# hasindu2008/cornetto

Measured on AMD Instinct MI355X. Metric: Gbases/s scanned (telowin+sdust+boringbits), higher is better.
Workload: dtype u8/u16 integer

## Files before the change

### cornetto_amd/csrc/common.hpp

```cpp
#pragma once
#include <hip/hip_runtime.h>

#include <cstdarg>
#include <cstdint>
#include <cstdio>
#include <cstdlib>
#include <cstring>
#include <algorithm>
#include <atomic>
#include <string>
#include <utility>
#include <vector>

#include "../../include/cornetto_accel.h"

#ifndef CN_STREAM_PRIO
#define CN_STREAM_PRIO 3
#endif

inline std::atomic<uint64_t> cn_uid_counter{1};

struct cornetto_accel {
    int device = 0;
    std::string tf_lut_key;
    const void *tf_lut_ptr = nullptr;
    uint64_t tf_bm_uid = 0;
    const void *tf_bm_ptr = nullptr;
    size_t tf_bm_words = 0;

    hipStream_t stream = nullptr;
    bool own_stream = false;
    hipStream_t stream2 = nullptr;
// ... 13 lines not shown
    Ws dev[64];
    Ws pin[32];
    int sd_slots = 0;
    int sd_cus = 0;
    int sift_per_cu = 0;
    int sift_per_cu_default = -1;
    int lazy = 0;
    hipStream_t copy_stream = nullptr;
    hipEvent_t ev_cp = nullptr;
    bool copies_pending = false;
    volatile int boost = 0;
    volatile unsigned long long launch_seq = 0;
    hipEvent_t ev3 = nullptr;
    int share = 100;
    int sd_stats = 0;
    struct SdPend {
        int state = 0;
        const void *a = nullptr;
        int32_t T = 0, W = 0;
        void *of = nullptr;
        size_t m_cap = 0, n_cap = 0, cap = 0;
        int64_t key = 0, n_done = 0;
        bool walk_pending = false;
    } sd_pend;
    unsigned long long sd_last[256] = {0};
    uint32_t scan_epoch = 0, scan_tickets = 0;
    uint32_t st_epoch = 0, st_tickets = 0;
    size_t te_cap = 0;
    int timing = 2;
};

static inline void *cn_ws(cornetto_accel_t *h, int slot, size_t bytes)
{
    cornetto_accel::Ws &w = h->dev[slot];
    if (bytes == 0) bytes = 16;
    if (w.bytes >= bytes) return w.p;
#ifdef CN_WS_ASYNC
    if (w.p) (void)hipFreeAsync(w.p, h->stream);
    w.p = nullptr;
    w.bytes = 0;
    const size_t want = bytes + bytes / 8;
    if (hipMallocAsync(&w.p, want, h->stream) == hipSuccess) w.bytes = want;
    else w.p = nullptr;
    return w.p;
#else
    if (w.p) (void)hipFree(w.p);
    w.p = nullptr;
// ... 296 lines not shown
```

### cornetto_amd/csrc/internal.hpp

```cpp
#pragma once
#include "common.hpp"

int cn_cov_prepare_impl(cornetto_accel_t *h, cornetto_cov_t *c, int32_t w, int32_t inc, uint64_t sums[3]);

struct CnCovSpec {
    bool queued = false;
    cornetto_regpk_t *o = nullptr;
    size_t n_copy = 0, cap = 0;
    unsigned long long *p_cnt = nullptr;
    uint32_t *p_cf = nullptr;
    int64_t key = 0;
};
int cn_cov_spec_queue(cornetto_accel_t *h, cornetto_cov_t *c, int32_t lo, int32_t hi, float low_mq, int32_t edge_len, int32_t min_ctg_len, int boring,
                      unsigned long long *p_cnt, CnCovSpec *S);
int cn_cov_spec_finish(cornetto_accel_t *h, cornetto_cov_t *c, CnCovSpec *S, cornetto_regpk_t **recs, int64_t *n_recs, int64_t **ctg_first);
int cn_cov_select_packed_impl(cornetto_accel_t *h, cornetto_cov_t *c, int32_t lo, int32_t hi, float low_mq, int32_t edge_len, int32_t min_ctg_len, int boring,
                              cornetto_regpk_t **recs, int64_t *n_recs, int64_t **ctg_first);

struct CnTeloSpec {
    bool queued = false;
    cornetto_hit_t *hits = nullptr;
    size_t hit_cap = 0;
    size_t seg_cap[4] = {0, 0, 0, 0};
    int4 *p_wins = nullptr;
    size_t win_cap = 0;
    unsigned long long *p_cnt = nullptr;
};
int cn_telo_spec_queue(cornetto_accel_t *h, cornetto_asm_t *a, const char *motif, double thr_adj, unsigned long long *p_cnt, CnTeloSpec *S);
int cn_telo_spec_finish(cornetto_accel_t *h, cornetto_asm_t *a, const char *motif, double thr_adj, CnTeloSpec *S, cornetto_hit_t **hits, int64_t *n_hits,
                        cornetto_win_t **wins, int64_t *n_wins);
int cn_telo_scan_impl(cornetto_accel_t *h, const cornetto_asm_t *a, const char *motif, double thr_adj, cornetto_hit_t **hits, int64_t *n_hits, cornetto_win_t **wins,
                      int64_t *n_wins);

int cn_telo_marks_impl(cornetto_accel_t *h, const cornetto_asm_t *a, const char *motif, const unsigned long long **d_marks);
```

### cornetto_amd/csrc/runtime.hip

```cpp
#include "common.hpp"
#include <chrono>
#include <condition_variable>
#include <deque>
#include <set>
#include <thread>

#include <map>
#include <mutex>
#include <unordered_map>

namespace {
std::mutex &g_pool_mu = *new std::mutex;
std::unordered_map<void *, size_t> &g_pool_live = *new std::unordered_map<void *, size_t>;
std::multimap<size_t, void *> &g_pool_free = *new std::multimap<size_t, void *>;
std::unordered_map<void *, uint64_t> &g_pool_age = *new std::unordered_map<void *, uint64_t>;
uint64_t g_pool_clock = 0;
constexpr size_t POOL_MIN = 1u << 20;
size_t g_pool_free_bytes = 0;
constexpr size_t POOL_KEEP_BYTES = 4ull << 30;
constexpr size_t POOL_KEEP = 12;
}

namespace {
std::condition_variable &g_pre_cv = *new std::condition_variable;
// ... 114 lines not shown
        }
    }
#endif
    cornetto_accel_t *h = new (std::nothrow) cornetto_accel;
    if (!h) return CORNETTO_E_NOMEM;
    h->device = device;
    if (stream) {
        h->stream = (hipStream_t)stream;
    } else {
        if (hipStreamCreateWithFlags(&h->stream, hipStreamNonBlocking) != hipSuccess) {
            delete h;
            return CORNETTO_E_NODEVICE;
        }
        h->own_stream = true;
    }
    *out = h;
    return CORNETTO_OK;
}

void cornetto_accel_close(cornetto_accel_t *h)
{
    if (!h) return;
    (void)hipSetDevice(h->device);
    (void)hipStreamSynchronize(h->stream);
    if (h->sd_pend.state != 0 && h->sd_pend.of) cornetto_free(h->sd_pend.of);
    h->sd_pend.state = 0;
    for (auto &r : h->recs) {
        (void)hipEventDestroy(r.a);
        (void)hipEventDestroy(r.b);
    }
    for (auto e : h->pool) (void)hipEventDestroy(e);
    for (auto &w : h->dev)
        if (w.p) (void)hipFree(w.p);
    for (auto &w : h->pin)
        if (w.p) (void)hipHostFree(w.p);
    if (h->ev1) (void)hipEventDestroy(h->ev1);
    if (h->ev2) (void)hipEventDestroy(h->ev2);
    if (h->ev3) (void)hipEventDestroy(h->ev3);
    if (h->copy_stream) {
        (void)hipStreamSynchronize(h->copy_stream);
        (void)hipStreamDestroy(h->copy_stream);
    }
    if (h->ev_cp) (void)hipEventDestroy(h->ev_cp);
    if (h->stream2) {
        (void)hipStreamSynchronize(h->stream2);
        (void)hipStreamDestroy(h->stream2);
    }
    if (h->own_stream) (void)hipStreamDestroy(h->stream);
    delete h;
// ... 77 lines not shown
    if (on && !h->copy_stream) {
        CN_HIP(h, hipSetDevice(h->device));
        CN_HIP(h, hipStreamCreateWithFlags(&h->copy_stream, hipStreamNonBlocking));
        CN_HIP(h, hipEventCreateWithFlags(&h->ev_cp, hipEventDisableTiming));
    }
    return CORNETTO_OK;
}

int cornetto_accel_wait(cornetto_accel_t *h)
{
    if (!h) return CORNETTO_E_ARG;
    if (h->copies_pending) {
        CN_HIP(h, hipSetDevice(h->device));
        CN_HIP(h, hipStreamSynchronize(h->copy_stream));
        h->copies_pending = false;
    }
    return CORNETTO_OK;
}

int cornetto_accel_boost(cornetto_accel_t *h, int on)
{
    if (!h) return CORNETTO_E_ARG;
    __atomic_store_n(&h->boost, on ? 1 : 0, __ATOMIC_RELEASE);
    return CORNETTO_OK;
}

int cornetto_accel_warm(cornetto_accel_t *h, int what)
{
    if (!h) return CORNETTO_E_ARG;
    const int32_t n = 4096;
    std::vector<uint8_t> seq((size_t)n);
    std::vector<uint16_t> d((size_t)n), q((size_t)n);
    uint32_t x = 12345u;
    for (int32_t i = 0; i < n; ++i) {
        x = x * 1664525u + 1013904223u;
        seq[(size_t)i] = "ACGT"[(x >> 24) & 3];
        d[(size_t)i] = (uint16_t)(20 + ((x >> 16) & 15));
        q[(size_t)i] = (uint16_t)(d[(size_t)i] >> ((i / 700) & 1));
    }
    for (int32_t i = 100; i < 700; ++i) seq[(size_t)i] = "TTAGGG"[(i - 100) % 6];
    for (int32_t i = 1000; i < 1100; ++i) seq[(size_t)i] = 'A';
    int rc = CORNETTO_OK;
    {
        CN_HIP(h, hipSetDevice(h->device));
        const size_t nb = (size_t)1 << 20;
        void *dv = cn_ws(h, WS_FQ_CNT, nb);
// ... 72 lines not shown
static const int64_t SLACK = 256;

static int asm_finish_table(cornetto_accel_t *h, cornetto_asm_t *a)
{
    size_t n = (size_t)(a->n > 0 ? a->n : 1);
    CN_HIP(h, hipMalloc((void **)&a->d_off, n * sizeof(int64_t)));
    CN_HIP(h, hipMalloc((void **)&a->d_len, n * sizeof(int32_t)));
    if (a->n) {
        CN_HIP(h, hipMemcpyAsync(a->d_off, a->off.data(), a->n * sizeof(int64_t), hipMemcpyHostToDevice, h->stream));
        CN_HIP(h, hipMemcpyAsync(a->d_len, a->len.data(), a->n * sizeof(int32_t), hipMemcpyHostToDevice, h->stream));
    }
    CN_HIP(h, hipStreamSynchronize(h->stream));
    if (a->total >= (64ll << 20)) {
        cn_result_prewarm((size_t)(a->total / 1536 + 1) * sizeof(cornetto_hit_t));
        cn_result_prewarm((size_t)(a->total / 4096 + 1) * sizeof(cornetto_ivl_t));
    }
    return CORNETTO_OK;
}

void cornetto_asm_free(cornetto_accel_t *h, cornetto_asm_t *a)
{
    if (!a) return;
    if (h) (void)hipSetDevice(h->device);
    if (h && h->sd_pend.state != 0 && h->sd_pend.a == a) {
        if (h->sd_pend.state == 1) (void)hipStreamSynchronize(h->stream);
        if (h->sd_pend.of) cornetto_free(h->sd_pend.of);
        h->sd_pend = cornetto_accel::SdPend{};
    }
    if (a->owned) (void)hipFree(a->owned);
    if (a->d_off) (void)hipFree(a->d_off);
    if (a->d_len) (void)hipFree(a->d_len);
    if (a->d_tf_tiles) (void)hipFree(a->d_tf_tiles);
    if (a->d_tf_ct0) (void)hipFree(a->d_tf_ct0);
    if (a->d_tw_boff) (void)hipFree(a->d_tw_boff);
    if (a->d_tw_tiles) (void)hipFree(a->d_tw_tiles);
    if (a->d_sd_chunks) (void)hipFree(a->d_sd_chunks);
    a->sd_pref.release(); a->tf_pref.release(); a->tw_pref.release();
    if (a->d_sd_walk) (void)hipFree(a->d_sd_walk);
    if (a->d_sd_plan) (void)hipFree(a->d_sd_plan);
    if (a->d_wtab) (void)hipFree(a->d_wtab);
    if (a->d_wtab_base) (void)hipFree(a->d_wtab_base);
    delete a;
}

int cornetto_asm_upload(cornetto_accel_t *h, const uint8_t *const *seqs, const int64_t *lens, int32_t n,
                        cornetto_asm_t **out)
{
    if (!h || !out || n < 0 || (n > 0 && (!seqs || !lens))) return cn_fail(h, CORNETTO_E_ARG, "asm_upload: bad argument");
    *out = nullptr;
    CN_HIP(h, hipSetDevice(h->device));
// ... 275 lines not shown
```

### cornetto_amd/csrc/scan.hpp

```cpp
#pragma once
#include "common.hpp"
#include "wave.hpp"

namespace cnscan {
namespace {

constexpr int SC_THREADS = 256;
constexpr int SC_ITEMS = 16;
constexpr int SC_TILE = SC_THREADS * SC_ITEMS;

template <typename T, int THREADS>
__device__ __forceinline__ T block_excl(T s, T &total)
{
    __shared__ T wtot[THREADS / 64];
    const int lane = threadIdx.x & 63, wv = threadIdx.x >> 6;
    const T inc = cnwave::wave_incl(s, lane);
    if (lane == 63) wtot[wv] = inc;
    __syncthreads();
    T pre = inc - s;
    total = 0;
#pragma unroll
    for (int w = 0; w < THREADS / 64; ++w) {
        if (w < wv) pre += wtot[w];
        total += wtot[w];
// ... 34 lines not shown
        for (int64_t pos = tile - 1;; pos -= 64) {
            const int64_t idx = pos - lane;
            unsigned long long x;
            for (;;) {
                x = idx >= 0 ? __hip_atomic_load(&st[idx * stride], __ATOMIC_RELAXED, __HIP_MEMORY_SCOPE_AGENT) : ((2ull << 62) | tag);
                const bool ready = (x >> 62) != 0 && (x & (0x3FFFFFFFull << 32)) == tag;
                if (__builtin_amdgcn_ballot_w64(!ready) == 0) break;
                __builtin_amdgcn_s_sleep(1);
            }
            const unsigned long long incl = __builtin_amdgcn_ballot_w64((x >> 62) == 2);
            const uint32_t val = (uint32_t)x;
            if (incl) {
                const int first = __builtin_ctzll(incl);
                excl += cnwave::wave_sum(lane <= first ? val : 0u);
                break;
            }
            excl += cnwave::wave_sum(val);
        }
    }
    if (lane == 0) __hip_atomic_store(&st[tile * stride], (2ull << 62) | tag | (excl + own), __ATOMIC_RELAXED, __HIP_MEMORY_SCOPE_AGENT);
    return excl;
}

struct Outs4 {
    uint32_t *o[4];
};
struct LbArgs {
    const uint32_t *in;
    int64_t n, np;
    int stride, m;
    Outs4 outs;
    unsigned long long *state;
    uint32_t *ticket;
    uint32_t ticket_base, epoch;
    unsigned long long *total;
};

__global__ __launch_bounds__(SC_THREADS) void scan_lookback(LbArgs A)
{
    __shared__ uint32_t s_gid, s_excl;
    const int t = threadIdx.x, lane = t & 63, wv = t >> 6;
    if (t == 0) s_gid = atomicAdd(A.ticket, 1u) - A.ticket_base;
    __syncthreads();
    const int64_t gid = s_gid;
    if (gid >= (int64_t)A.m * A.np) return;
    const int q = (int)(gid / A.np);
// ... 1 lines not shown
    const int64_t base = tile * SC_TILE + (int64_t)t * SC_ITEMS;
    uint32_t v[SC_ITEMS], bt;
    uint32_t pre = tile_excl(A.in + q, base, A.n, A.stride, v, bt);
    if (wv == 0) {
        const uint32_t excl = lookback_excl(A.state + (int64_t)q * A.np, 1, tile, A.epoch, bt, lane);
        if (lane == 0) {
            s_excl = excl;
            if (A.total && tile == A.np - 1) A.total[q] = (unsigned long long)excl + bt;
        }
    }
    __syncthreads();
    pre += s_excl;
    tile_write(A.outs.o[q], base, A.n, pre, v);
}

static inline int exclusive_u32_multi(cornetto_accel_t *h, const char *name, const uint32_t *in, int64_t n, int stride, int m, uint32_t *const *outs,
                                      unsigned long long *d_total)
{
    if (n <= 0 || m <= 0) return CORNETTO_OK;
    if (m > 4) m = 4;
    Outs4 o{};
    for (int q = 0; q < m; ++q) o.o[q] = outs[q];
    const int64_t np = (n + SC_TILE - 1) / SC_TILE;
    const size_t need = 64 + (size_t)m * (size_t)np * 8;
    const bool fresh = h->dev[WS_SCAN].bytes < need || h->scan_epoch >= 0x3FFFFFFFu;
    uint8_t *ws = (uint8_t *)cn_ws(h, WS_SCAN, need);
    if (!ws) return cn_fail(h, CORNETTO_E_NOMEM, "scan: workspace allocation failed");
    const int rc = [&]() -> int {
        if (fresh) {
            CN_HIP(h, hipMemsetAsync(ws, 0, h->dev[WS_SCAN].bytes, h->stream));
            h->scan_tickets = 0;
            h->scan_epoch = 0;
        }
        const uint32_t epoch = h->scan_epoch + 1;
        LbArgs A{in, n, np, stride, m, o, reinterpret_cast<unsigned long long *>(ws + 64), reinterpret_cast<uint32_t *>(ws), h->scan_tickets, epoch, d_total};
        CN_LAUNCH(h, name, scan_lookback<<<dim3((unsigned)(m * np)), dim3(SC_THREADS), 0, h->stream>>>(A));
        h->scan_epoch = epoch;
        h->scan_tickets += (uint32_t)(m * np);
        return CORNETTO_OK;
    }();
    if (rc != CORNETTO_OK) h->dev[WS_SCAN].bytes = 0;
    return rc;
}

static inline int exclusive_u32(cornetto_accel_t *h, const char *name, const uint32_t *in, int64_t n, int stride, uint32_t *out, unsigned long long *d_total)
{
    return exclusive_u32_multi(h, name, in, n, stride, 1, &out, d_total);
}

}
}
```

### cornetto_amd/csrc/sdust.hip

```cpp
#include <algorithm>
#include <type_traits>
#include <ctime>
#include <sched.h>

#include "common.hpp"
#include "scan.hpp"
#include "tiles.hpp"
#include "ivlmerge.hpp"

namespace {

__device__ __forceinline__ int nt4_code(uint32_t c);
struct SdArgs;
struct SdChunk;
template <bool LEAN = false>
__device__ int sd_find_start(const SdArgs &A, const SdChunk ch, const uint8_t *seq);

struct SdChunk {
    int32_t ctg, start, end;
};
struct SdChunkFill {
    SdChunk *out;
    const int32_t *len;
    int32_t chunk;
    __device__ void operator()(int64_t t, int c, int64_t j) const
    {
        const int64_t s = j * chunk, e = s + chunk;
        out[t] = SdChunk{c, (int32_t)s, (int32_t)(e < len[c] ? e : len[c])};
    }
};

// ... 1290 lines not shown
    if (flag[c]) {
        pos = r * S;
    } else {
        if (S > 1u && j < H * (S - 1u)) pos = (j / (S - 1u)) * S + 1u + j % (S - 1u);
        else pos = H * S + (j - H * (S - 1u));
    }
    perm[pos] = (uint32_t)c;
}

__global__ void sdust_gather(const uint2 *in, const uint32_t *cnt, const uint32_t *dst_off, uint32_t cap, const SdChunk *chunks,
                             int32_t n_chunks, cornetto_ivl_t *dst, uint32_t dst_cap = 0xFFFFFFFFu)
{
    const int cid = blockIdx.x * blockDim.x + threadIdx.x;
    if (cid >= n_chunks) return;
    uint32_t n = cnt[cid];
    if (n == 0) return;
    if (n > cap) n = cap;
    const int32_t ctg = chunks[cid].ctg;
    const uint2 *src = in + (size_t)cid * cap;
    const uint32_t o = dst_off[cid];
    for (uint32_t i = 0; i < n && o + i < dst_cap; ++i) dst[o + i] = cornetto_ivl_t{ctg, (int32_t)src[i].x, (int32_t)src[i].y};
}

__global__ void sd_sample_count(const uint8_t *bases, const int64_t *ctg_off, const int32_t *ctg_len, unsigned long long *count)
{
    const int c = blockIdx.y;
    const int len = ctg_len[c];
    const uint8_t *seq = bases + ctg_off[c];
    unsigned n = 0;
    for (long long s = (long long)blockIdx.x * blockDim.x + threadIdx.x; s * 2048 + 64 <= len; s += (long long)gridDim.x * blockDim.x)
        n += sd_sample_heavy(SdChunk{c, (int32_t)(s * 2048), (int32_t)std::min<long long>(len, s * 2048 + 2048)}, seq);
    const unsigned long long m = sd_ballot(n != 0);
    (void)m;
    for (int d = 32; d > 0; d >>= 1) n += __shfl_down(n, d);
    if ((threadIdx.x & 63) == 0 && n) atomicAdd(count, (unsigned long long)n);
}

__global__ void sd_make_order(const uint32_t *walk, const uint32_t *iswalk, const uint32_t *rank, int32_t n_chunks, uint32_t *order)
{
    const int k = blockIdx.x * blockDim.x + threadIdx.x;
    if (k >= n_chunks) return;
    const uint32_t nw = walk[0];
    if ((uint32_t)k < nw) order[k] = walk[2 + k];
    if (!iswalk[k]) order[nw + (uint32_t)k - rank[k]] = (uint32_t)k;
}

}

extern "C" {

}

namespace {
int sd_one_go_finish(cornetto_accel_t *h, cornetto_asm_t *a, cornetto_ivl_t *of, unsigned long long *p_tot, size_t cap, size_t n_cap, size_t m_cap, int64_t key,
                     bool walk_pending, cornetto_ivl_t **ivls, int64_t *n_ivls)
{
    if (hipStreamSynchronize(h->stream) != hipSuccess) {
        cornetto_free(of);
        return cn_fail(h, CORNETTO_E_HIP, "sdust: stitch / copy back failed");
    }
    const uint32_t ovf_f = (uint32_t)(p_tot[1] & 0xFFFFFFFFull);
    const bool wtab_f = (p_tot[1] >> 32) != 0;
    const unsigned long long rows_f = p_tot[0], out_f = rows_f ? p_tot[9] : 0ull;
    if (!wtab_f && ovf_f <= cap && rows_f <= n_cap && out_f != ~0ull && out_f <= m_cap && out_f <= rows_f && (rows_f == 0 || out_f > 0)) {
        if (walk_pending) a->sd_walk_key = key;
        a->sd_est_rows = (int64_t)rows_f;
        a->sd_est_out = (int64_t)out_f;
        cn_timing_end(h);
        *ivls = of;
        *n_ivls = (int64_t)out_f;
        return 0;
    }
    cornetto_free(of);
    a->sd_est_key = -1;
    return 1;
}

int sdust_asm_impl(cornetto_accel_t *h, const cornetto_asm_t *a_in, int32_t T, int32_t W, cornetto_ivl_t **ivls, int64_t *n_ivls, const int phase)
{
    static const bool trace = CN_DEV_INT("CORNETTO_SDUST_TRACE", 0) != 0;
    struct timespec ts0;
    clock_gettime(CLOCK_MONOTONIC, &ts0);
    auto stamp = [&](const char *what) {
        if (!trace) return;
        struct timespec t;
        clock_gettime(CLOCK_MONOTONIC, &t);
        fprintf(stderr, "[sdust trace] %-22s %8.3f ms\n", what, (t.tv_sec - ts0.tv_sec) * 1e3 + (t.tv_nsec - ts0.tv_nsec) * 1e-6);
    };
    if (!h || !a_in || !ivls || !n_ivls) return cn_fail(h, CORNETTO_E_ARG, "sdust: bad argument");
    cornetto_asm_t *a = const_cast<cornetto_asm_t *>(a_in);
    *ivls = nullptr;
    *n_ivls = 0;
    if (W < 3 || W > 1026) return cn_fail(h, CORNETTO_E_UNSUPPORTED, "sdust: -w %d outside 3..1026 (the reference crashes below 3)", W);
    if (T < 0 || T > (1 << 20)) return cn_fail(h, CORNETTO_E_UNSUPPORTED, "sdust: -t %d outside 0..2^20", T);
    CN_HIP(h, hipSetDevice(h->device));
    cn_timing_begin(h);

    const int variant0 = CN_DEV_INT("CORNETTO_SDUST_VARIANT", 0);
    const bool w64_path = W - 2 <= 64 && T >= 5 && T <= 100000 && variant0 == 0;
    if (w64_path && h->sd_slots == 0) {
// ... 150 lines not shown
    const size_t nc = (size_t)a->sd_n_chunks;
    cornetto_ivl_t *o = nullptr;
    int64_t n_out = 0;
    stamp("chunk table");
    if (nc > 0) {
        const SdChunk *d_chunks = reinterpret_cast<const SdChunk *>(a->d_sd_chunks);
        uint32_t *d_cnt = (uint32_t *)cn_ws(h, WS_SD_CNT, nc * 8 + 4);
        unsigned long long *d_tot = (unsigned long long *)cn_ws(h, WS_SD_STATS, 2048 + 64 * 64);
        unsigned long long *p_tot = (unsigned long long *)cn_pin(h, PIN_SMALL, 2048);
        if (!d_cnt || !d_tot || !p_tot) return cn_fail(h, CORNETTO_E_NOMEM, "sdust: workspace allocation failed");
        uint32_t *d_off = d_cnt + nc;
        stamp("small workspaces");
        const bool env_stats = CN_DEV_INT("CORNETTO_SDUST_STATS", 0) != 0;
        const bool want_stats = env_stats || h->sd_stats != 0;
        size_t cap = (size_t)std::max<int64_t>(16, chunk / 32);
        cap = (size_t)CN_DEV_INT("CORNETTO_SDUST_CAP", (int)cap);
        if (h->dev[WS_SD_OUT].bytes / (nc * sizeof(uint2)) > cap) cap = h->dev[WS_SD_OUT].bytes / (nc * sizeof(uint2));
        unsigned long long tot = 0;
        uint2 *d_out = nullptr;
        const int64_t est_key = key * 131 + T * 1031 + W;
        const bool one_go = w64_path && sift_on && !want_stats && a->sd_est_key == est_key && a->sd_est_rows >= 0 && CN_DEV_INT("CORNETTO_SDUST_FUSED", 1);
        if (phase == 1 && !one_go)
            return CORNETTO_OK;
        for (int attempt = 0; attempt < 4; ++attempt) {
            d_out = (uint2 *)cn_ws(h, WS_SD_OUT, nc * cap * sizeof(uint2));
            if (!d_out) return cn_fail(h, CORNETTO_E_NOMEM, "sdust: workspace allocation of %zu bytes failed", nc * cap * sizeof(uint2));
            CN_HIP(h, hipMemsetAsync(d_tot, 0, 2048 + 64 * 64, h->stream));
            uint32_t *d_slots = (uint32_t *)cn_ws(h, WS_SD_OFF, (size_t)(std::max<int64_t>(sd_waves, 1) + SD_WPB) * 64 * 64 * sizeof(uint32_t));
            if (!d_slots) return cn_fail(h, CORNETTO_E_NOMEM, "sdust: workspace allocation failed");
            stamp("row + slot workspaces");
            const bool use_w64 = w64_path;
            SdArgs A{a->d_bases, a->d_off, a->d_len, d_chunks, (int32_t)nc, T, W, d_out, d_cnt, (uint32_t)cap,
                     want_stats ? d_tot + 2 : nullptr, reinterpret_cast<uint32_t *>(d_tot + 1), d_slots, nullptr,
                     reinterpret_cast<uint32_t *>(d_tot + 8), nullptr, 0, CN_DEV_INT("CORNETTO_SDUST_RUNON", 1), (int32_t)chunk, a->d_wtab, a->d_wtab_base, reinterpret_cast<uint32_t *>(d_tot + 1) + 1};
            unsigned nb = (unsigned)((nc + 63) / 64);
            bool sift_walk_pending = false;
            bool dense_pending = false;
            struct DenseJoin {
                cornetto_accel_t *h;
                bool *pending;
                ~DenseJoin() { if (*pending && h->stream2) (void)hipStreamSynchronize(h->stream2); }
            } dense_join{h, &dense_pending};
            if (use_w64 && sift_on) {
                CN_HIP(h, hipMemsetAsync(d_cnt, 0, nc * 4, h->stream));
                const uint32_t reg_cap = (uint32_t)(chunk + 128);
                const uint32_t lds_wave = sift_lds_bytes(reg_cap);
                int lmin = 1;
                while (5 * (lmin + 1) <= T && lmin < 16) ++lmin;
                const bool walk_known = a->d_sd_walk && a->sd_walk_key == key;
                const size_t walk_words = 2 + 4 * nc + 2;
                if (!walk_known) {
                    if (a->d_sd_walk) { (void)hipFree(a->d_sd_walk); a->d_sd_walk = nullptr; }
                    a->sd_walk_key = -1;
                    if (cn_obj_malloc(h, (void **)&a->d_sd_walk, walk_words * 4) != hipSuccess) return cn_fail(h, CORNETTO_E_NOMEM, "sdust: device allocation failed");
                    CN_HIP(h, hipMemsetAsync(a->d_sd_walk, 0, (2 + 2 * nc) * 4, h->stream));
                }
                uint32_t *d_wflag = a->d_sd_walk + 2 + nc, *d_wrank = d_wflag + nc, *d_worder = d_wrank + nc;
                SiftArgs S{a->d_bases, a->d_off, a->d_len, d_chunks, (int32_t)nc, T, W, lds_wave, reg_cap,
                           walk_known ? d_worder : nullptr, walk_known ? nullptr : a->d_sd_walk, walk_known ? nullptr : d_wflag,
                           reinterpret_cast<uint32_t *>(d_tot + 256), T / 10 + 1, lmin, CN_DEV_INT("CORNETTO_SIFT_ABL", 0),
                           std::min(65, std::max(1, CN_DEV_INT("CORNETTO_SIFT_DP", 24))), std::min(65, std::max(1, CN_DEV_INT("CORNETTO_SIFT_L2SKIP", 48)))};
                sift_walk_pending = !walk_known;
                SdArgs R = A;
                R.stats = want_stats ? d_tot + 200 : nullptr;
                const bool cap_default = reg_cap == SIFT_CAP_DEFAULT && !CN_DEV_INT("CORNETTO_SIFT_GENERIC", 0) && !CN_DEV_INT("CORNETTO_SIFT_ABL", 0);
                if (h->sift_per_cu == 0 || h->sift_per_cu_default != (cap_default ? 1 : 0)) {
                    int per_cu = 0;
                    const hipError_t oe = cap_default ? hipOccupancyMaxActiveBlocksPerMultiprocessor(&per_cu, sd_sift<false, SIFT_CAP_DEFAULT>, 64 * SIFT_WPB, lds_wave * SIFT_WPB)
                                                      : hipOccupancyMaxActiveBlocksPerMultiprocessor(&per_cu, sd_sift<false>, 64 * SIFT_WPB, lds_wave * SIFT_WPB);
                    if (oe != hipSuccess || per_cu < 1) per_cu = 8;
                    h->sift_per_cu = per_cu;
                    h->sift_per_cu_default = cap_default ? 1 : 0;
                }
                const int per_cu_all = std::max(1, std::min<int>(h->sift_per_cu, (int)(163840 / ((lds_wave * SIFT_WPB + 1279) / 1280 * 1280))));
                const bool free_now = __atomic_load_n(&h->boost, __ATOMIC_ACQUIRE) != 0;
                const size_t cus_n = (size_t)std::max(h->sd_cus, 1);
                const size_t slots_all = (size_t)per_cu_all * cus_n;
                const size_t slots = free_now ? slots_all : std::max<size_t>(cus_n, slots_all * (size_t)h->share / 100);
                const size_t all_blocks = (nc + SIFT_WPB - 1) / SIFT_WPB;
                const unsigned nbk = (unsigned)std::min<size_t>(all_blocks, (size_t)CN_DEV_INT("CORNETTO_SIFT_BLOCKS", (int)slots));
                const unsigned extra = (unsigned)std::min<size_t>(all_blocks > nbk ? all_blocks - nbk : 0, slots_all > slots ? slots_all - slots : 0);
                const bool may_help = phase == 0 && extra > 0 && !want_stats && h->share < CN_DEV_INT("CORNETTO_SDUST_HELP_BELOW", 70);
                if (may_help) {
                    if (!h->stream2) {
                        int pr_least = 0, pr_greatest = 0;
                        (void)hipDeviceGetStreamPriorityRange(&pr_least, &pr_greatest);
                        CN_HIP(h, hipStreamCreateWithPriority(&h->stream2, hipStreamNonBlocking, pr_greatest));
                        CN_HIP(h, hipEventCreateWithFlags(&h->ev2, hipEventDisableTiming));
                        CN_HIP(h, hipEventCreateWithFlags(&h->ev1, hipEventDisableTiming));
                    }
                    if (!h->ev3) CN_HIP(h, hipEventCreateWithFlags(&h->ev3, hipEventDisableTiming));
                    CN_HIP(h, hipEventRecord(h->ev1, h->stream));
                }
                stamp("set up");
                if (want_stats) CN_LAUNCH(h, "sdust_kernel", sd_sift<true><<<dim3(nbk), dim3(64 * SIFT_WPB), lds_wave * SIFT_WPB, h->stream>>>(S, R));
                else if (cap_default) CN_LAUNCH(h, "sdust_kernel", sd_sift<false, SIFT_CAP_DEFAULT><<<dim3(nbk), dim3(64 * SIFT_WPB), lds_wave * SIFT_WPB, h->stream>>>(S, R));
                else CN_LAUNCH(h, "sdust_kernel", sd_sift<false><<<dim3(nbk), dim3(64 * SIFT_WPB), lds_wave * SIFT_WPB, h->stream>>>(S, R));
                __atomic_fetch_add(&h->launch_seq, 1ull, __ATOMIC_RELEASE);
                if (may_help) {
                    CN_HIP(h, hipEventRecord(h->ev3, h->stream));
                    bool helped = false;
                    while (hipEventQuery(h->ev3) == hipErrorNotReady) {
                        if (!helped && __atomic_load_n(&h->boost, __ATOMIC_ACQUIRE) != 0) {
                            CN_HIP(h, hipStreamWaitEvent(h->stream2, h->ev1, 0));
                            if (cap_default) sd_sift<false, SIFT_CAP_DEFAULT><<<dim3(extra), dim3(64 * SIFT_WPB), lds_wave * SIFT_WPB, h->stream2>>>(S, R);
                            else sd_sift<false><<<dim3(extra), dim3(64 * SIFT_WPB), lds_wave * SIFT_WPB, h->stream2>>>(S, R);
                            dense_pending = true;
                            CN_HIP(h, hipGetLastError());
                            CN_HIP(h, hipEventRecord(h->ev2, h->stream2));
                            helped = true;
                        }
                        sched_yield();
                    }
                    if (helped) CN_HIP(h, hipStreamWaitEvent(h->stream, h->ev2, 0));
// ... 97 lines not shown
                if ((unsigned)sd_waves < nb) nb = (unsigned)sd_waves;
                nb = (nb + SD_WPB - 1) / SD_WPB * SD_WPB;
                if (want_stats) CN_LAUNCH(h, "sdust_kernel", sdust_w64<true><<<dim3(nb / SD_WPB), dim3(64 * SD_WPB), 0, h->stream>>>(A));
                else CN_LAUNCH(h, "sdust_kernel", sdust_w64<false><<<dim3(nb / SD_WPB), dim3(64 * SD_WPB), 0, h->stream>>>(A));
            } else if (W - 2 <= 64) {
                CN_LAUNCH(h, "sdust_kernel", sdust_kernel<64><<<dim3(nb), dim3(64), 0, h->stream>>>(A));
            } else if (W - 2 <= 255) {
                CN_LAUNCH(h, "sdust_kernel", sdust_kernel<256><<<dim3(nb), dim3(64), 0, h->stream>>>(A));
            } else {
                int rc = 512;
                while (rc < W - 2) rc <<= 1;
                const size_t NL = (size_t)nb * 64;
                uint8_t *g = (uint8_t *)cn_ws(h, WS_SD_OFF, NL * ((size_t)rc * 5 + 512) + 64);
                if (!g) return cn_fail(h, CORNETTO_E_NOMEM, "sdust: workspace allocation of %zu bytes failed", NL * ((size_t)rc * 5 + 512));
                uint32_t *g_cw = reinterpret_cast<uint32_t *>(g), *g_cv = g_cw + 64 * NL, *g_slot = g_cv + 64 * NL;
                uint8_t *g_ring = reinterpret_cast<uint8_t *>(g_slot + (size_t)rc * NL);
                CN_LAUNCH(h, "sdust_kernel", sdust_kernel_g<<<dim3(nb), dim3(64), 0, h->stream>>>(A, g_ring, g_cw, g_cv, g_slot, rc));
            }
            if (!sift_on) __atomic_fetch_add(&h->launch_seq, 1ull, __ATOMIC_RELEASE);
            if (dense_pending) {
                CN_HIP(h, hipStreamWaitEvent(h->stream, h->ev2, 0));
                dense_pending = false;
            }
            CN_TRY(cnscan::exclusive_u32(h, "sdust_scan", d_cnt, (int64_t)nc, 1, d_off, d_tot));
            if (one_go) {
                size_t n_cap = (size_t)(a->sd_est_rows + a->sd_est_rows / 8 + 4096);
                if (CN_DEV_INT("CORNETTO_SDUST_EST_FORCE", 0) > 0) n_cap = (size_t)CN_DEV_INT("CORNETTO_SDUST_EST_FORCE", 0);
                const size_t m_cap = (size_t)(a->sd_est_out + a->sd_est_out / 16 + 1024);
                uint8_t *ws = (uint8_t *)cn_ws(h, WS_SD_DST, 2 * n_cap * sizeof(cornetto_ivl_t) + cnivl::ws_bytes(n_cap));
                cornetto_ivl_t *of = (cornetto_ivl_t *)cn_result_alloc(std::max<size_t>(m_cap * sizeof(cornetto_ivl_t), (size_t)1 << 20));
                if (ws && of && n_cap < 0x7fffffffull) {
                    cornetto_ivl_t *d_dst = (cornetto_ivl_t *)(ws + cnivl::ws_bytes(n_cap)), *d_st = d_dst + n_cap;
                    const unsigned nbg = (unsigned)((nc + 255) / 256);
                    CN_LAUNCH(h, "sdust_gather", sdust_gather<<<dim3(nbg), dim3(256), 0, h->stream>>>(d_out, d_cnt, d_off, (uint32_t)cap, d_chunks, (int32_t)nc, d_dst, (uint32_t)n_cap));
                    CN_HIP(h, hipMemsetAsync(d_tot + 9, 0xFF, 8, h->stream));
                    int rcf = cnivl::merge_fused(h, "sdust_stitch", d_dst, d_tot, (int64_t)n_cap, 0, d_st, d_tot + 9);
                    if (rcf != CORNETTO_OK) { cornetto_free(of); return rcf; }
                    stamp("tail queued");
                    if (hipMemcpyAsync(of, d_st, m_cap * sizeof(cornetto_ivl_t), hipMemcpyDeviceToHost, h->stream) != hipSuccess ||
                        hipMemcpyAsync(p_tot, d_tot, 128, hipMemcpyDeviceToHost, h->stream) != hipSuccess) {
                        (void)hipStreamSynchronize(h->stream);
                        cornetto_free(of);
                        return cn_fail(h, CORNETTO_E_HIP, "sdust: stitch / copy back failed");
                    }
                    if (phase == 1) {
                        h->sd_pend.state = 1; h->sd_pend.a = a; h->sd_pend.T = T; h->sd_pend.W = W; h->sd_pend.of = of;
                        h->sd_pend.m_cap = m_cap; h->sd_pend.n_cap = n_cap; h->sd_pend.cap = cap; h->sd_pend.key = key; h->sd_pend.walk_pending = sift_walk_pending;
                        return CORNETTO_OK;
                    }
                    const int fin = sd_one_go_finish(h, a, of, p_tot, cap, n_cap, m_cap, key, sift_walk_pending, ivls, n_ivls);
                    if (fin <= 0) {
                        if (fin == 0) stamp("results on the host (one go)");
                        return fin;
                    }
                } else if (of) {
                    cornetto_free(of);
                }
            }
            stamp("main kernel queued");
            CN_HIP(h, hipMemcpyAsync(p_tot, d_tot, want_stats ? 2048 : 128, hipMemcpyDeviceToHost, h->stream));
            CN_HIP(h, hipStreamSynchronize(h->stream));
            stamp("main kernel done");
            if (want_stats) {
                memcpy(h->sd_last, p_tot, 2048);
                if (a->sd_flagged >= 0) h->sd_last[7] = (unsigned long long)a->sd_flagged;
                h->sd_last[254] = nb;
                h->sd_last[255] = nc;
            }
            if (env_stats)
                for (int b = 0; b < 32; ++b)
                    if (p_tot[16 + 4 * b])
                        fprintf(stderr, "[sdust stats]   waves that ran %4.1f-%4.1f ms: %6llu, job fetches %llu, find_perfect calls %llu (%llu with candidates)\n", b * 0.5, b * 0.5 + 0.5,
                                p_tot[16 + 4 * b], p_tot[18 + 4 * b], p_tot[19 + 4 * b], p_tot[17 + 4 * b]);
            if (env_stats && sift_on)
                fprintf(stderr, "[sdust stats] sift: tiles %llu, positions with ct > T/10 %llu, after L1 %llu, after L2 %llu; resolve: steps %llu, window reads %llu (behind a gap of 2 / 3-4 / 5-8: %llu / %llu / %llu), dp tiles %llu; passes with candidates %llu; base-by-base steps of chunks with other bytes %llu\n",
                        p_tot[206], p_tot[203], p_tot[204], p_tot[205], p_tot[200], p_tot[201], p_tot[209], p_tot[210], p_tot[211], p_tot[208], p_tot[202], p_tot[207]);
            if (env_stats)
                fprintf(stderr, "[sdust stats] flagged low-complexity %llu; chunks %zu waves %u wave-steps %llu find_perfect calls %llu (%llu with candidates) plain groups %llu; wave time avg %.1f us max %.1f us; queue: %.1f fetch rounds and %.1f us per wave\n", p_tot[7], nc, nb,
                        p_tot[2], p_tot[3], p_tot[10], p_tot[4], nb ? (double)p_tot[5] / nb / 100.0 : 0.0, (double)p_tot[6] / 100.0, nb ? (double)p_tot[11] / nb : 0.0, nb ? (double)p_tot[12] / nb / 100.0 : 0.0);
            const uint32_t ovf = (uint32_t)(p_tot[1] & 0xFFFFFFFFull);
            const bool need_wtab = (p_tot[1] >> 32) != 0;
// ... 76 lines not shown
{
    if (h && h->sd_pend.state != 0) {
        cornetto_ivl_t *dv = nullptr;
        int64_t dn = 0;
        if (cornetto_sdust_asm_end(h, reinterpret_cast<const cornetto_asm_t *>(h->sd_pend.a), h->sd_pend.T, h->sd_pend.W, &dv, &dn) == CORNETTO_OK) cornetto_free(dv);
    }
    return sdust_asm_impl(h, a_in, T, W, ivls, n_ivls, 0);
}

int cornetto_sdust_asm_begin(cornetto_accel_t *h, const cornetto_asm_t *a_in, int32_t T, int32_t W)
{
    if (!h || !a_in) return cn_fail(h, CORNETTO_E_ARG, "sdust: bad argument");
    if (h->sd_pend.state != 0) return cn_fail(h, CORNETTO_E_ARG, "sdust: cornetto_sdust_asm_begin() twice without cornetto_sdust_asm_end()");
    cornetto_ivl_t *dv = nullptr;
    int64_t dn = 0;
    return sdust_asm_impl(h, a_in, T, W, &dv, &dn, 1);
}

int cornetto_sdust_asm_end(cornetto_accel_t *h, const cornetto_asm_t *a_in, int32_t T, int32_t W, cornetto_ivl_t **ivls, int64_t *n_ivls)
{
    if (!h || !a_in || !ivls || !n_ivls) return cn_fail(h, CORNETTO_E_ARG, "sdust: bad argument");
    *ivls = nullptr;
    *n_ivls = 0;
    const cornetto_accel::SdPend P = h->sd_pend;
    h->sd_pend = cornetto_accel::SdPend{};
    if (P.state != 0 && (P.a != a_in || P.T != T || P.W != W)) {
        if (P.state == 2) cornetto_free(P.of);
        else { (void)hipSetDevice(h->device); (void)hipStreamSynchronize(h->stream); cornetto_free(P.of); }
        return sdust_asm_impl(h, a_in, T, W, ivls, n_ivls, 0);
    }
    if (P.state == 2) {
        *ivls = (cornetto_ivl_t *)P.of;
        *n_ivls = P.n_done;
        return CORNETTO_OK;
    }
    if (P.state == 1) {
        CN_HIP(h, hipSetDevice(h->device));
        unsigned long long *p_tot = (unsigned long long *)cn_pin(h, PIN_SMALL, 2048);
        if (!p_tot) return cn_fail(h, CORNETTO_E_NOMEM, "sdust: workspace allocation failed");
        const int fin = sd_one_go_finish(h, const_cast<cornetto_asm_t *>(a_in), (cornetto_ivl_t *)P.of, p_tot, P.cap, P.n_cap, P.m_cap, P.key, P.walk_pending, ivls, n_ivls);
        if (fin <= 0) return fin;
    }
    return sdust_asm_impl(h, a_in, T, W, ivls, n_ivls, 0);
}

int cornetto_accel_sdust_stats(cornetto_accel_t *h, int enable, uint64_t *out, int cap)
{
    if (!h) return CORNETTO_E_ARG;
    h->sd_stats = enable ? 1 : 0;
    int n = 0;
    if (out)
        for (; n < cap && n < 256; ++n) out[n] = h->sd_last[n];
    return n;
}

static cornetto_accel_t *g_handle = nullptr;

struct cornetto_sdust_buf {
    uint64_t *res;
    int64_t cap;
};

cornetto_sdust_buf_t *cornetto_sdust_buf_init(void *km)
// ... 56 lines not shown
```

Baseline: 485.9.

## Fuse sdust scan with gather, skip count memset, defer tail for boosted widening

The separate exclusive scan and gather kernels in the sdust one-go path become a single decoupled-lookback scan+gather kernel. That kernel also zeroes the per-chunk counters, so the next call can skip the counter memset when the workspace is unchanged. In the asynchronous begin phase the tail work is deferred so that a later boost call can launch extra sift blocks on a second stream before queuing the tail. This removes one launch, one memset and one extra pass over the counts, at the cost of mutex locking and more complex pending-state handling.

```diff
diff --git a/cornetto_amd/csrc/common.hpp b/cornetto_amd/csrc/common.hpp
--- a/cornetto_amd/csrc/common.hpp
+++ b/cornetto_amd/csrc/common.hpp
@@ -8,6 +8,7 @@
 #include <cstring>
 #include <algorithm>
 #include <atomic>
+#include <mutex>
 #include <string>
 #include <utility>
 #include <vector>
@@ -67,7 +68,15 @@
         size_t m_cap = 0, n_cap = 0, cap = 0;
         int64_t key = 0, n_done = 0;
         bool walk_pending = false;
+        void *late = nullptr;
+        bool helped = false;
+        int late_rc = 0;
+        const void *cnt_ptr = nullptr;
+        size_t cnt_n = 0;
     } sd_pend;
+    std::mutex sd_mu;
+    const void *sd_cnt_ptr = nullptr;
+    size_t sd_cnt_bytes = 0, sd_cnt_zero = 0;
     unsigned long long sd_last[256] = {0};
     uint32_t scan_epoch = 0, scan_tickets = 0;
     uint32_t st_epoch = 0, st_tickets = 0;
diff --git a/cornetto_amd/csrc/internal.hpp b/cornetto_amd/csrc/internal.hpp
--- a/cornetto_amd/csrc/internal.hpp
+++ b/cornetto_amd/csrc/internal.hpp
@@ -33,3 +33,6 @@
                       int64_t *n_wins);
 
 int cn_telo_marks_impl(cornetto_accel_t *h, const cornetto_asm_t *a, const char *motif, const unsigned long long **d_marks);
+
+int cn_sd_queue_rest(cornetto_accel_t *h, bool widen);
+void cn_sd_drop_late(cornetto_accel_t *h);
diff --git a/cornetto_amd/csrc/runtime.hip b/cornetto_amd/csrc/runtime.hip
--- a/cornetto_amd/csrc/runtime.hip
+++ b/cornetto_amd/csrc/runtime.hip
@@ -1,4 +1,5 @@
 #include "common.hpp"
+#include "internal.hpp"
 #include <chrono>
 #include <condition_variable>
 #include <deque>
@@ -160,9 +161,14 @@
 {
     if (!h) return;
     (void)hipSetDevice(h->device);
-    (void)hipStreamSynchronize(h->stream);
-    if (h->sd_pend.state != 0 && h->sd_pend.of) cornetto_free(h->sd_pend.of);
-    h->sd_pend.state = 0;
+    {
+        std::lock_guard<std::mutex> lk(h->sd_mu);
+        cn_sd_drop_late(h);
+        (void)hipStreamSynchronize(h->stream);
+        if (h->stream2) (void)hipStreamSynchronize(h->stream2);
+        if (h->sd_pend.state != 0 && h->sd_pend.of) cornetto_free(h->sd_pend.of);
+        h->sd_pend = cornetto_accel::SdPend{};
+    }
     for (auto &r : h->recs) {
         (void)hipEventDestroy(r.a);
         (void)hipEventDestroy(r.b);
@@ -286,6 +292,10 @@
 {
     if (!h) return CORNETTO_E_ARG;
     __atomic_store_n(&h->boost, on ? 1 : 0, __ATOMIC_RELEASE);
+    if (on) {
+        std::lock_guard<std::mutex> lk(h->sd_mu);
+        (void)cn_sd_queue_rest(h, true);
+    }
     return CORNETTO_OK;
 }
 
@@ -404,10 +414,17 @@
 {
     if (!a) return;
     if (h) (void)hipSetDevice(h->device);
-    if (h && h->sd_pend.state != 0 && h->sd_pend.a == a) {
-        if (h->sd_pend.state == 1) (void)hipStreamSynchronize(h->stream);
-        if (h->sd_pend.of) cornetto_free(h->sd_pend.of);
-        h->sd_pend = cornetto_accel::SdPend{};
+    if (h) {
+        std::lock_guard<std::mutex> lk(h->sd_mu);
+        if (h->sd_pend.state != 0 && h->sd_pend.a == a) {
+            cn_sd_drop_late(h);
+            if (h->sd_pend.state == 1) {
+                (void)hipStreamSynchronize(h->stream);
+                if (h->sd_pend.helped && h->stream2) (void)hipStreamSynchronize(h->stream2);
+            }
+            if (h->sd_pend.of) cornetto_free(h->sd_pend.of);
+            h->sd_pend = cornetto_accel::SdPend{};
+        }
     }
     if (a->owned) (void)hipFree(a->owned);
     if (a->d_off) (void)hipFree(a->d_off);
diff --git a/cornetto_amd/csrc/scan.hpp b/cornetto_amd/csrc/scan.hpp
--- a/cornetto_amd/csrc/scan.hpp
+++ b/cornetto_amd/csrc/scan.hpp
@@ -80,6 +80,29 @@
     return excl;
 }
 
+template <class F>
+static inline int with_states(cornetto_accel_t *h, int64_t tiles, F &&launch)
+{
+    const size_t need = 64 + (size_t)tiles * 8;
+    const bool fresh = h->dev[WS_SCAN].bytes < need || h->scan_epoch >= 0x3FFFFFFFu;
+    uint8_t *ws = (uint8_t *)cn_ws(h, WS_SCAN, need);
+    if (!ws) return cn_fail(h, CORNETTO_E_NOMEM, "scan: workspace allocation failed");
+    const int rc = [&]() -> int {
+        if (fresh) {
+            CN_HIP(h, hipMemsetAsync(ws, 0, h->dev[WS_SCAN].bytes, h->stream));
+            h->scan_tickets = 0;
+            h->scan_epoch = 0;
+        }
+        const uint32_t epoch = h->scan_epoch + 1;
+        CN_TRY(launch(reinterpret_cast<unsigned long long *>(ws + 64), reinterpret_cast<uint32_t *>(ws), h->scan_tickets, epoch));
+        h->scan_epoch = epoch;
+        h->scan_tickets += (uint32_t)tiles;
+        return CORNETTO_OK;
+    }();
+    if (rc != CORNETTO_OK) h->dev[WS_SCAN].bytes = 0;
+    return rc;
+}
+
 struct Outs4 {
     uint32_t *o[4];
 };
@@ -127,25 +150,11 @@
     Outs4 o{};
     for (int q = 0; q < m; ++q) o.o[q] = outs[q];
     const int64_t np = (n + SC_TILE - 1) / SC_TILE;
-    const size_t need = 64 + (size_t)m * (size_t)np * 8;
-    const bool fresh = h->dev[WS_SCAN].bytes < need || h->scan_epoch >= 0x3FFFFFFFu;
-    uint8_t *ws = (uint8_t *)cn_ws(h, WS_SCAN, need);
-    if (!ws) return cn_fail(h, CORNETTO_E_NOMEM, "scan: workspace allocation failed");
-    const int rc = [&]() -> int {
-        if (fresh) {
-            CN_HIP(h, hipMemsetAsync(ws, 0, h->dev[WS_SCAN].bytes, h->stream));
-            h->scan_tickets = 0;
-            h->scan_epoch = 0;
-        }
-        const uint32_t epoch = h->scan_epoch + 1;
-        LbArgs A{in, n, np, stride, m, o, reinterpret_cast<unsigned long long *>(ws + 64), reinterpret_cast<uint32_t *>(ws), h->scan_tickets, epoch, d_total};
+    return with_states(h, (int64_t)m * np, [&](unsigned long long *state, uint32_t *ticket, uint32_t ticket_base, uint32_t epoch) -> int {
+        LbArgs A{in, n, np, stride, m, o, state, ticket, ticket_base, epoch, d_total};
         CN_LAUNCH(h, name, scan_lookback<<<dim3((unsigned)(m * np)), dim3(SC_THREADS), 0, h->stream>>>(A));
-        h->scan_epoch = epoch;
-        h->scan_tickets += (uint32_t)(m * np);
         return CORNETTO_OK;
-    }();
-    if (rc != CORNETTO_OK) h->dev[WS_SCAN].bytes = 0;
-    return rc;
+    });
 }
 
 static inline int exclusive_u32(cornetto_accel_t *h, const char *name, const uint32_t *in, int64_t n, int stride, uint32_t *out, unsigned long long *d_total)
diff --git a/cornetto_amd/csrc/sdust.hip b/cornetto_amd/csrc/sdust.hip
--- a/cornetto_amd/csrc/sdust.hip
+++ b/cornetto_amd/csrc/sdust.hip
@@ -7,6 +7,7 @@
 #include "scan.hpp"
 #include "tiles.hpp"
 #include "ivlmerge.hpp"
+#include "internal.hpp"
 
 namespace {
 
@@ -1343,6 +1344,54 @@
     for (uint32_t i = 0; i < n && o + i < dst_cap; ++i) dst[o + i] = cornetto_ivl_t{ctg, (int32_t)src[i].x, (int32_t)src[i].y};
 }
 
+struct SgArgs {
+    const uint2 *in;
+    uint32_t *cnt;
+    uint32_t cap;
+    const SdChunk *chunks;
+    int32_t n_chunks;
+    cornetto_ivl_t *dst;
+    uint32_t dst_cap;
+    unsigned long long *state;
+    uint32_t *ticket;
+    uint32_t ticket_base, epoch;
+    unsigned long long *total, *marker;
+};
+__global__ __launch_bounds__(cnscan::SC_THREADS) void sdust_scan_gather(SgArgs A)
+{
+    __shared__ uint32_t s_tile, s_excl;
+    const int t = threadIdx.x, lane = t & 63, wv = t >> 6;
+    if (t == 0) s_tile = atomicAdd(A.ticket, 1u) - A.ticket_base;
+    __syncthreads();
+    const int64_t tile = s_tile, n = A.n_chunks, np = (n + cnscan::SC_TILE - 1) / cnscan::SC_TILE;
+    if (tile >= np) return;
+    const int64_t base = tile * cnscan::SC_TILE + (int64_t)t * cnscan::SC_ITEMS;
+    uint32_t v[cnscan::SC_ITEMS], bt;
+    uint32_t o = cnscan::tile_excl(A.cnt, base, n, 1, v, bt);
+    if (wv == 0) {
+        const uint32_t excl = cnscan::lookback_excl(A.state, 1, tile, A.epoch, bt, lane);
+        if (lane == 0) {
+            s_excl = excl;
+            if (tile == np - 1) *A.total = (unsigned long long)excl + bt;
+            if (tile == 0) *A.marker = ~0ull;
+        }
+    }
+    __syncthreads();
+    o += s_excl;
+#pragma unroll 1
+    for (int k = 0; k < cnscan::SC_ITEMS; ++k) {
+        const int64_t cid = base + k;
+        uint32_t m = v[k];
+        if (m == 0) continue;
+        A.cnt[cid] = 0;
+        if (m > A.cap) m = A.cap;
+        const int32_t ctg = A.chunks[cid].ctg;
+        const uint2 *src = A.in + (size_t)cid * A.cap;
+        for (uint32_t i = 0; i < m && o + i < A.dst_cap; ++i) A.dst[o + i] = cornetto_ivl_t{ctg, (int32_t)src[i].x, (int32_t)src[i].y};
+        o += v[k];
+    }
+}
+
 __global__ void sd_sample_count(const uint8_t *bases, const int64_t *ctg_off, const int32_t *ctg_len, unsigned long long *count)
 {
     const int c = blockIdx.y;
@@ -1373,10 +1422,43 @@
 }
 
 namespace {
+struct SdTail {
+    const uint2 *d_out;
+    uint32_t *d_cnt;
+    const SdChunk *d_chunks;
+    size_t nc, cap, n_cap, m_cap;
+    unsigned long long *d_tot, *p_tot;
+    cornetto_ivl_t *d_dst, *d_st, *of;
+};
+struct SdLate {
+    SiftArgs S;
+    SdArgs R;
+    unsigned extra;
+    uint32_t lds_wave;
+    bool cap_default;
+    SdTail tail;
+};
+
+int sd_queue_tail(cornetto_accel_t *h, const SdTail &t)
+{
+    const int64_t np = ((int64_t)t.nc + cnscan::SC_TILE - 1) / cnscan::SC_TILE;
+    CN_TRY(cnscan::with_states(h, np, [&](unsigned long long *state, uint32_t *ticket, uint32_t ticket_base, uint32_t epoch) -> int {
+        SgArgs G{t.d_out, t.d_cnt, (uint32_t)t.cap, t.d_chunks, (int32_t)t.nc, t.d_dst, (uint32_t)t.n_cap, state, ticket, ticket_base, epoch, t.d_tot, t.d_tot + 9};
+        CN_LAUNCH(h, "sdust_gather", sdust_scan_gather<<<dim3((unsigned)np), dim3(cnscan::SC_THREADS), 0, h->stream>>>(G));
+        return CORNETTO_OK;
+    }));
+    CN_TRY(cnivl::merge_fused(h, "sdust_stitch", t.d_dst, t.d_tot, (int64_t)t.n_cap, 0, t.d_st, t.d_tot + 9));
+    if (hipMemcpyAsync(t.of, t.d_st, t.m_cap * sizeof(cornetto_ivl_t), hipMemcpyDeviceToHost, h->stream) != hipSuccess ||
+        hipMemcpyAsync(t.p_tot, t.d_tot, 128, hipMemcpyDeviceToHost, h->stream) != hipSuccess)
+        return cn_fail(h, CORNETTO_E_HIP, "sdust: stitch / copy back failed");
+    return CORNETTO_OK;
+}
+
 int sd_one_go_finish(cornetto_accel_t *h, cornetto_asm_t *a, cornetto_ivl_t *of, unsigned long long *p_tot, size_t cap, size_t n_cap, size_t m_cap, int64_t key,
-                     bool walk_pending, cornetto_ivl_t **ivls, int64_t *n_ivls)
+                     bool walk_pending, bool helped, const void *cnt_ptr, size_t cnt_n, cornetto_ivl_t **ivls, int64_t *n_ivls)
 {
     if (hipStreamSynchronize(h->stream) != hipSuccess) {
+        if (helped && h->stream2) (void)hipStreamSynchronize(h->stream2);
         cornetto_free(of);
         return cn_fail(h, CORNETTO_E_HIP, "sdust: stitch / copy back failed");
     }
@@ -1387,16 +1469,53 @@
         if (walk_pending) a->sd_walk_key = key;
         a->sd_est_rows = (int64_t)rows_f;
         a->sd_est_out = (int64_t)out_f;
+        if (cnt_ptr && cnt_ptr == h->dev[WS_SD_CNT].p) {
+            h->sd_cnt_ptr = cnt_ptr;
+            h->sd_cnt_bytes = h->dev[WS_SD_CNT].bytes;
+            h->sd_cnt_zero = cnt_n;
+        }
         cn_timing_end(h);
         *ivls = of;
         *n_ivls = (int64_t)out_f;
         return 0;
     }
+    if (helped && h->stream2) (void)hipStreamSynchronize(h->stream2);
     cornetto_free(of);
     a->sd_est_key = -1;
     return 1;
 }
-
+}
+
+int cn_sd_queue_rest(cornetto_accel_t *h, bool widen)
+{
+    cornetto_accel::SdPend &P = h->sd_pend;
+    if (P.state != 1 || !P.late) return CORNETTO_OK;
+    SdLate *L = static_cast<SdLate *>(P.late);
+    P.late = nullptr;
+    P.late_rc = [&]() -> int {
+        CN_HIP(h, hipSetDevice(h->device));
+        if (widen && L->extra > 0) {
+            CN_HIP(h, hipStreamWaitEvent(h->stream2, h->ev1, 0));
+            if (L->cap_default) sd_sift<false, SIFT_CAP_DEFAULT><<<dim3(L->extra), dim3(64 * SIFT_WPB), L->lds_wave * SIFT_WPB, h->stream2>>>(L->S, L->R);
+            else sd_sift<false><<<dim3(L->extra), dim3(64 * SIFT_WPB), L->lds_wave * SIFT_WPB, h->stream2>>>(L->S, L->R);
+            P.helped = true;
+            CN_HIP(h, hipGetLastError());
+            CN_HIP(h, hipEventRecord(h->ev2, h->stream2));
+            CN_HIP(h, hipStreamWaitEvent(h->stream, h->ev2, 0));
+        }
+        return sd_queue_tail(h, L->tail);
+    }();
+    delete L;
+    return P.late_rc;
+}
+
+void cn_sd_drop_late(cornetto_accel_t *h)
+{
+    delete static_cast<SdLate *>(h->sd_pend.late);
+    h->sd_pend.late = nullptr;
+}
+
+namespace {
 int sdust_asm_impl(cornetto_accel_t *h, const cornetto_asm_t *a_in, int32_t T, int32_t W, cornetto_ivl_t **ivls, int64_t *n_ivls, const int phase)
 {
     static const bool trace = CN_DEV_INT("CORNETTO_SDUST_TRACE", 0) != 0;
@@ -1593,10 +1712,13 @@
         const bool one_go = w64_path && sift_on && !want_stats && a->sd_est_key == est_key && a->sd_est_rows >= 0 && CN_DEV_INT("CORNETTO_SDUST_FUSED", 1);
         if (phase == 1 && !one_go)
             return CORNETTO_OK;
+        bool go = one_go;
         for (int attempt = 0; attempt < 4; ++attempt) {
             d_out = (uint2 *)cn_ws(h, WS_SD_OUT, nc * cap * sizeof(uint2));
             if (!d_out) return cn_fail(h, CORNETTO_E_NOMEM, "sdust: workspace allocation of %zu bytes failed", nc * cap * sizeof(uint2));
             CN_HIP(h, hipMemsetAsync(d_tot, 0, 2048 + 64 * 64, h->stream));
+            const bool cnt_zero = d_cnt == h->sd_cnt_ptr && h->dev[WS_SD_CNT].bytes == h->sd_cnt_bytes && nc <= h->sd_cnt_zero;
+            h->sd_cnt_zero = 0;
             uint32_t *d_slots = (uint32_t *)cn_ws(h, WS_SD_OFF, (size_t)(std::max<int64_t>(sd_waves, 1) + SD_WPB) * 64 * 64 * sizeof(uint32_t));
             if (!d_slots) return cn_fail(h, CORNETTO_E_NOMEM, "sdust: workspace allocation failed");
             stamp("row + slot workspaces");
@@ -1607,13 +1729,15 @@
             unsigned nb = (unsigned)((nc + 63) / 64);
             bool sift_walk_pending = false;
             bool dense_pending = false;
+            SdLate late{};
+            late.extra = 0;
             struct DenseJoin {
                 cornetto_accel_t *h;
                 bool *pending;
                 ~DenseJoin() { if (*pending && h->stream2) (void)hipStreamSynchronize(h->stream2); }
             } dense_join{h, &dense_pending};
             if (use_w64 && sift_on) {
-                CN_HIP(h, hipMemsetAsync(d_cnt, 0, nc * 4, h->stream));
+                if (!cnt_zero) CN_HIP(h, hipMemsetAsync(d_cnt, 0, nc * 4, h->stream));
                 const uint32_t reg_cap = (uint32_t)(chunk + 128);
                 const uint32_t lds_wave = sift_lds_bytes(reg_cap);
                 int lmin = 1;
@@ -1652,7 +1776,11 @@
                 const unsigned nbk = (unsigned)std::min<size_t>(all_blocks, (size_t)CN_DEV_INT("CORNETTO_SIFT_BLOCKS", (int)slots));
                 const unsigned extra = (unsigned)std::min<size_t>(all_blocks > nbk ? all_blocks - nbk : 0, slots_all > slots ? slots_all - slots : 0);
                 const bool may_help = phase == 0 && extra > 0 && !want_stats && h->share < CN_DEV_INT("CORNETTO_SDUST_HELP_BELOW", 70);
-                if (may_help) {
+                const bool widen = phase == 1 && go && extra > 0 && walk_known;
+                if (widen) {
+                    late.S = S; late.R = R; late.extra = extra; late.lds_wave = lds_wave; late.cap_default = cap_default;
+                }
+                if (may_help || widen) {
                     if (!h->stream2) {
                         int pr_least = 0, pr_greatest = 0;
                         (void)hipDeviceGetStreamPriorityRange(&pr_least, &pr_greatest);
@@ -1660,7 +1788,7 @@
                         CN_HIP(h, hipEventCreateWithFlags(&h->ev2, hipEventDisableTiming));
                         CN_HIP(h, hipEventCreateWithFlags(&h->ev1, hipEventDisableTiming));
                     }
-                    if (!h->ev3) CN_HIP(h, hipEventCreateWithFlags(&h->ev3, hipEventDisableTiming));
+                    if (may_help && !h->ev3) CN_HIP(h, hipEventCreateWithFlags(&h->ev3, hipEventDisableTiming));
                     CN_HIP(h, hipEventRecord(h->ev1, h->stream));
                 }
                 stamp("set up");
@@ -1804,8 +1932,7 @@
                 CN_HIP(h, hipStreamWaitEvent(h->stream, h->ev2, 0));
                 dense_pending = false;
             }
-            CN_TRY(cnscan::exclusive_u32(h, "sdust_scan", d_cnt, (int64_t)nc, 1, d_off, d_tot));
-            if (one_go) {
+            if (go) {
                 size_t n_cap = (size_t)(a->sd_est_rows + a->sd_est_rows / 8 + 4096);
                 if (CN_DEV_INT("CORNETTO_SDUST_EST_FORCE", 0) > 0) n_cap = (size_t)CN_DEV_INT("CORNETTO_SDUST_EST_FORCE", 0);
                 const size_t m_cap = (size_t)(a->sd_est_out + a->sd_est_out / 16 + 1024);
@@ -1813,32 +1940,43 @@
                 cornetto_ivl_t *of = (cornetto_ivl_t *)cn_result_alloc(std::max<size_t>(m_cap * sizeof(cornetto_ivl_t), (size_t)1 << 20));
                 if (ws && of && n_cap < 0x7fffffffull) {
                     cornetto_ivl_t *d_dst = (cornetto_ivl_t *)(ws + cnivl::ws_bytes(n_cap)), *d_st = d_dst + n_cap;
-                    const unsigned nbg = (unsigned)((nc + 255) / 256);
-                    CN_LAUNCH(h, "sdust_gather", sdust_gather<<<dim3(nbg), dim3(256), 0, h->stream>>>(d_out, d_cnt, d_off, (uint32_t)cap, d_chunks, (int32_t)nc, d_dst, (uint32_t)n_cap));
-                    CN_HIP(h, hipMemsetAsync(d_tot + 9, 0xFF, 8, h->stream));
-                    int rcf = cnivl::merge_fused(h, "sdust_stitch", d_dst, d_tot, (int64_t)n_cap, 0, d_st, d_tot + 9);
-                    if (rcf != CORNETTO_OK) { cornetto_free(of); return rcf; }
-                    stamp("tail queued");
-                    if (hipMemcpyAsync(of, d_st, m_cap * sizeof(cornetto_ivl_t), hipMemcpyDeviceToHost, h->stream) != hipSuccess ||
-                        hipMemcpyAsync(p_tot, d_tot, 128, hipMemcpyDeviceToHost, h->stream) != hipSuccess) {
+                    const SdTail tail{d_out, d_cnt, d_chunks, nc, cap, n_cap, m_cap, d_tot, p_tot, d_dst, d_st, of};
+                    cornetto_accel::SdPend pend;
+                    pend.state = 1; pend.a = a; pend.T = T; pend.W = W; pend.of = of;
+                    pend.m_cap = m_cap; pend.n_cap = n_cap; pend.cap = cap; pend.key = key; pend.walk_pending = sift_walk_pending;
+                    pend.cnt_ptr = d_cnt; pend.cnt_n = nc;
+                    if (phase == 1 && late.extra > 0) {
+                        late.tail = tail;
+                        pend.late = new SdLate(late);
+                        std::lock_guard<std::mutex> lk(h->sd_mu);
+                        h->sd_pend = pend;
+                        return CORNETTO_OK;
+                    }
+                    const int rcf = sd_queue_tail(h, tail);
+                    if (rcf != CORNETTO_OK) {
                         (void)hipStreamSynchronize(h->stream);
                         cornetto_free(of);
-                        return cn_fail(h, CORNETTO_E_HIP, "sdust: stitch / copy back failed");
-                    }
+                        return rcf;
+                    }
+                    stamp("tail queued");
                     if (phase == 1) {
-                        h->sd_pend.state = 1; h->sd_pend.a = a; h->sd_pend.T = T; h->sd_pend.W = W; h->sd_pend.of = of;
-                        h->sd_pend.m_cap = m_cap; h->sd_pend.n_cap = n_cap; h->sd_pend.cap = cap; h->sd_pend.key = key; h->sd_pend.walk_pending = sift_walk_pending;
+                        std::lock_guard<std::mutex> lk(h->sd_mu);
+                        h->sd_pend = pend;
                         return CORNETTO_OK;
                     }
-                    const int fin = sd_one_go_finish(h, a, of, p_tot, cap, n_cap, m_cap, key, sift_walk_pending, ivls, n_ivls);
+                    const int fin = sd_one_go_finish(h, a, of, p_tot, cap, n_cap, m_cap, key, sift_walk_pending, false, d_cnt, nc, ivls, n_ivls);
                     if (fin <= 0) {
                         if (fin == 0) stamp("results on the host (one go)");
                         return fin;
                     }
-                } else if (of) {
-                    cornetto_free(of);
-                }
-            }
+                    go = false;
+                    --attempt;
+                    continue;
+                }
+                if (of) cornetto_free(of);
+                go = false;
+            }
+            CN_TRY(cnscan::exclusive_u32(h, "sdust_scan", d_cnt, (int64_t)nc, 1, d_off, d_tot));
             stamp("main kernel queued");
             CN_HIP(h, hipMemcpyAsync(p_tot, d_tot, want_stats ? 2048 : 128, hipMemcpyDeviceToHost, h->stream));
             CN_HIP(h, hipStreamSynchronize(h->stream));
@@ -1961,11 +2099,25 @@
     if (!h || !a_in || !ivls || !n_ivls) return cn_fail(h, CORNETTO_E_ARG, "sdust: bad argument");
     *ivls = nullptr;
     *n_ivls = 0;
-    const cornetto_accel::SdPend P = h->sd_pend;
-    h->sd_pend = cornetto_accel::SdPend{};
+    cornetto_accel::SdPend P;
+    {
+        std::lock_guard<std::mutex> lk(h->sd_mu);
+        if (h->sd_pend.state == 1 && h->sd_pend.late) {
+            (void)hipSetDevice(h->device);
+            if (h->sd_pend.a == a_in && h->sd_pend.T == T && h->sd_pend.W == W) (void)cn_sd_queue_rest(h, false);
+            else cn_sd_drop_late(h);
+        }
+        P = h->sd_pend;
+        h->sd_pend = cornetto_accel::SdPend{};
+    }
     if (P.state != 0 && (P.a != a_in || P.T != T || P.W != W)) {
         if (P.state == 2) cornetto_free(P.of);
-        else { (void)hipSetDevice(h->device); (void)hipStreamSynchronize(h->stream); cornetto_free(P.of); }
+        else {
+            (void)hipSetDevice(h->device);
+            (void)hipStreamSynchronize(h->stream);
+            if (P.helped && h->stream2) (void)hipStreamSynchronize(h->stream2);
+            cornetto_free(P.of);
+        }
         return sdust_asm_impl(h, a_in, T, W, ivls, n_ivls, 0);
     }
     if (P.state == 2) {
@@ -1975,9 +2127,16 @@
     }
     if (P.state == 1) {
         CN_HIP(h, hipSetDevice(h->device));
+        if (P.late_rc != CORNETTO_OK) {
+            (void)hipStreamSynchronize(h->stream);
+            if (P.helped && h->stream2) (void)hipStreamSynchronize(h->stream2);
+            cornetto_free(P.of);
+            return P.late_rc;
+        }
         unsigned long long *p_tot = (unsigned long long *)cn_pin(h, PIN_SMALL, 2048);
         if (!p_tot) return cn_fail(h, CORNETTO_E_NOMEM, "sdust: workspace allocation failed");
-        const int fin = sd_one_go_finish(h, const_cast<cornetto_asm_t *>(a_in), (cornetto_ivl_t *)P.of, p_tot, P.cap, P.n_cap, P.m_cap, P.key, P.walk_pending, ivls, n_ivls);
+        const int fin = sd_one_go_finish(h, const_cast<cornetto_asm_t *>(a_in), (cornetto_ivl_t *)P.of, p_tot, P.cap, P.n_cap, P.m_cap, P.key, P.walk_pending, P.helped,
+                                         P.cnt_ptr, P.cnt_n, ivls, n_ivls);
         if (fin <= 0) return fin;
     }
     return sdust_asm_impl(h, a_in, T, W, ivls, n_ivls, 0);
```

Measured after the change: 488.6, median of 6. No clear change (+0.6%).
